# fatimp/SIFT3D

Measured on AMD Instinct MI355X. Metric: Mvoxel/s detect+describe (float32 volume resident in HBM), higher is better.
Workload: dtype f32; 1 GPU; 512x512x512 float32 lattice-blob volume, detect+describe, default parameters (sigma0 1.6, sigma_n 1.15, 3 levels/octave); parallelism=single GPU

## Files before the change

include/sift3d_amd.h:

```cpp
#ifndef SIFT3D_AMD_H
#define SIFT3D_AMD_H

#include <stddef.h>
#include <stdint.h>

#include "sift3d/imtypes.h"

#ifdef __cplusplus
extern "C" {
#endif

#define SIFT3D_AMD_API __attribute__((visibility("default")))


SIFT3D_AMD_API int
sift3d_amd_detect_keypoints_device(sift3d_detector *det, const float *d_volume,
                                   int nx, int ny, int nz, double ux, double uy,
                                   double uz, sift3d_keypoint_store *store);

SIFT3D_AMD_API int
sift3d_amd_image_set_units(sift3d_image *im, double ux, double uy, double uz);

SIFT3D_AMD_API int
sift3d_amd_detector_set_cuboid_extrema(sift3d_detector *det, int on);
// ... 308 lines not shown
SIFT3D_AMD_API int sift3d_hip_memcpy_d2d(void *d_dst, const void *d_src, size_t bytes, void *stream);
SIFT3D_AMD_API int sift3d_hip_memcpy2d_d2h(void *h_dst, size_t dst_pitch, const void *d_src,
                                           size_t src_pitch, size_t width, size_t height, void *stream);
SIFT3D_AMD_API int sift3d_hip_stream_wait_event(void *stream, void *ev);
SIFT3D_AMD_API int sift3d_hip_rows_scatter(float *d_dst, const void *d_all, size_t blk_bytes,
                                           const uint32_t *d_map, uint32_t n, void *stream);
SIFT3D_AMD_API int sift3d_hip_max_rows(float *d_dst, const float *d_rows, int nrows, int n, void *stream);
SIFT3D_AMD_API int sift3d_hip_memset(void *d_dst, int byte, size_t bytes, void *stream);
SIFT3D_AMD_API void *sift3d_hip_stream_create(void);
SIFT3D_AMD_API void *sift3d_hip_stream_create_high(void);
SIFT3D_AMD_API void sift3d_hip_stream_destroy(void *stream);
SIFT3D_AMD_API int sift3d_hip_stream_sync(void *stream);
SIFT3D_AMD_API void *sift3d_hip_event_create(void);
SIFT3D_AMD_API void sift3d_hip_event_destroy(void *ev);
SIFT3D_AMD_API int sift3d_hip_event_record(void *ev, void *stream);
SIFT3D_AMD_API double sift3d_hip_event_elapsed_ms(void *ev_start, void *ev_stop);


SIFT3D_AMD_API int
sift3d_hip_absmax(const float *d_src, size_t n, float *d_max, void *stream);

SIFT3D_AMD_API int
sift3d_hip_scale(const float *d_src, float *d_dst, size_t n, const float *d_max,
                 void *stream);

#define SIFT3D_HIP_MAX_TAPS 65

typedef struct {
    const float *src;
    float *dst;
    int nx, ny, nz;
    int axis;
    int width;
    const float *taps;
    float unit_factor;
    int n_glob, off;
    int z_lo, z_hi;
    int variant;
} sift3d_hip_fir_args;

SIFT3D_AMD_API int
sift3d_hip_fir(const sift3d_hip_fir_args *args, void *stream);
SIFT3D_AMD_API int
sift3d_hip_fir_x_scaled(const sift3d_hip_fir_args *args, const float *d_max, void *stream);
SIFT3D_AMD_API int sift3d_hip_fir_x_scaled_covers(const sift3d_hip_fir_args *args);

SIFT3D_AMD_API int
sift3d_hip_fir_yz_u1(const float *d_src, float *d_dst, int nx, int ny, int nz, const float *taps,
                     int width, int n_glob, int off, int z_lo, int z_hi, void *stream);
SIFT3D_AMD_API int sift3d_hip_fir_yz_u1_covers(const float *d_src, const float *d_dst, int nx, int ny,
                                               int width, int n_glob);

SIFT3D_AMD_API int
sift3d_hip_subtract_absmax(const float *d_a, const float *d_b, float *d_dst, size_t n,
                           float *d_absmax, void *stream);

#define SIFT3D_HIP_MAX_DOG_STACK 8
SIFT3D_AMD_API int sift3d_hip_dog_stack(const float *const *d_g, float *const *d_d, int n_gauss,
                                        size_t n, float *d_absmax, void *stream);

SIFT3D_AMD_API int
sift3d_hip_downsample2(const float *d_src, int nx, int ny, float *d_dst, int mx, int my,
                       int mz, void *stream);

typedef struct {
    const float *prev, *cur, *next;
    const float *d_absmax;
    int z_lo, z_hi;
    int tag;
} sift3d_hip_extrema_level;

typedef struct {
    uint32_t idx;
    int32_t tag;
    float val;
} sift3d_hip_cand;

SIFT3D_AMD_API size_t
sift3d_hip_extrema_work_bytes(int nx, int ny, int nz, int nlevels);
SIFT3D_AMD_API int
sift3d_hip_extrema(const sift3d_hip_extrema_level *levels, int nlevels, int nx, int ny,
                   int nz, double peak_thresh, sift3d_hip_cand *d_out, uint32_t cap,
                   uint32_t *d_count, void *d_work, size_t work_bytes, void *stream);

SIFT3D_AMD_API int
sift3d_hip_extrema_mode(const sift3d_hip_extrema_level *levels, int nlevels, int nx, int ny, int nz,
                        double peak_thresh, int cuboid, sift3d_hip_cand *d_out, uint32_t cap,
                        uint32_t *d_count, void *d_work, size_t work_bytes, void *stream);

SIFT3D_AMD_API int sift3d_hip_dogmax_stack(const float *const *d_g, int n_gauss, size_t n,
                                           float *d_absmax, void *stream);
SIFT3D_AMD_API int
sift3d_hip_extrema_gauss6(const float *const *d_g, const float *d_absmax, int nx, int ny, int nz,
                          int z_lo, int z_hi, int tag0, double peak_thresh, sift3d_hip_cand *d_out,
                          uint32_t cap, uint32_t *d_count, void *d_work, size_t work_bytes,
                          void *stream);
SIFT3D_AMD_API int
sift3d_hip_extrema_gauss6_phase(const float *const *d_g, const float *d_absmax, int nx, int ny, int nz,
                                int z_lo, int z_hi, int tag0, double peak_thresh, sift3d_hip_cand *d_out,
                                uint32_t cap, uint32_t *d_count, void *d_work, size_t work_bytes,
                                void *stream, int phase);
SIFT3D_AMD_API int sift3d_hip_dogmax_sub(const float *const *d_g, int nx, int ny, int nz, float *d_est,
                                         void *stream);
typedef struct {
    const float *const *d_g;
    int nx, ny, nz;
// ... 100 lines not shown
```

profiles/pmc_fir.py:

```python
#!/usr/bin/env python3
import csv
import glob
import json
import os
import sys

ROOT = os.path.dirname(os.path.dirname(os.path.abspath(__file__)))
sys.path.insert(0, ROOT)


def _require_built():
    lib = os.environ.get("SIFT3D_AMD_LIB") or os.path.join(ROOT, "sift3d_amd", "libsift3d_amd.so")
    if not os.path.exists(lib):
        sys.exit("%s is missing -- build first: python3 -c \"from sift3d_amd import _native; "
                 "_native.build()\"" % lib)

SIG = [0.5387011637869722, 0.9732939207323564, 1.2262734984654078, 1.5450077936447955,
       1.9465878414647133, 2.4525469969308156]


def run_guarded(*a, **k):
    _require_built()
    return run(*a, **k)


def run(n=512, reps=3):
    import torch
    from sift3d_amd import api, hip
    src = torch.empty((n, n, n), device="cuda")
    dst = torch.empty_like(src)
    hip.synth_lattice(src, 0, 11)
    for s in SIG:
        taps = api.gauss_filter(s)
        for ax in range(3):
            for _ in range(reps):
                hip.fir(src, dst, ax, taps)
        for _ in range(reps):
            hip.fir_yz(src, dst, taps)
    torch.cuda.synchronize()


def run_pyramid(n=512, builds=2):
    import torch
    from sift3d_amd import api, hip
    _require_built()
    vol = torch.empty((n, n, n), device="cuda")
    hip.synth_lattice(vol, 0, 11)
    torch.cuda.synchronize()
    det = api.Detector()
    for _ in range(builds):
        assert det.build_pyramid_device(vol.data_ptr(), n, n, n) == 0
    torch.cuda.synchronize()


def parse_pyramid(fetch_dir, write_dir, n=512, builds=2):
    def total(d, name):
        tot, by = 0.0, {}
        for f in glob.glob(os.path.join(d, "**", "*counter_collection.csv"), recursive=True):
            for r in csv.DictReader(open(f)):
                if r["Counter_Name"] != name or "synth" in r["Kernel_Name"]:
                    continue
                k = r["Kernel_Name"].split("(")[0].replace("void ", "")
                v = float(r["Counter_Value"])
                tot += v
                by[k] = by.get(k, 0.0) + v
        return tot, by
    fe, fby = total(fetch_dir, "FETCH_SIZE")
    wr, wby = total(write_dir, "WRITE_SIZE")
    num_oct = 0
    m = n
    alg = 0
    while m >= 8:
        alg += 24 * m ** 3 * (6 if num_oct == 0 else 5)
        num_oct += 1
        m //= 2
    hbm = (2.0 * fe + wr) * 1024.0 / builds
    by = {k: round((2.0 * fby.get(k, 0.0) + wby.get(k, 0.0)) * 1024.0 / builds) for k in set(fby) | set(wby)}
    return dict(hbm_bytes=round(hbm), algorithmic_bytes=alg, ratio=round(hbm / alg, 3), builds=builds,
                note="every kernel of sift3d_amd_build_pyramid_device (max|v|, all FIR passes of all octaves, "
                     "down-sampling): (2 * FETCH_SIZE + WRITE_SIZE) * 1024 summed over its dispatches",
                hbm_bytes_by_kernel=dict(sorted(by.items(), key=lambda kv: -kv[1])))


def parse(fetch_dir, write_dir, n=512):
    def load(d, name):
        out = {}
        for f in glob.glob(os.path.join(d, "**", "*counter_collection.csv"), recursive=True):
            for r in csv.DictReader(open(f)):
                if r["Counter_Name"] != name:
                    continue
                k = r["Kernel_Name"].split("(")[0].replace("void ", "")
                gx = int(r["Grid_Size_X"]) if "Grid_Size_X" in r else 0
                out.setdefault((k, gx), []).append(float(r["Counter_Value"]))
        return out
    fe, wr = load(fetch_dir, "FETCH_SIZE"), load(write_dir, "WRITE_SIZE")
    res = {}
    for (k, gx), v in fe.items():
        if "fir" not in k:
            continue
        w = wr.get((k, gx), [0.0])
        fetch_b = 2.0 * 1024.0 * sum(v) / len(v)
        write_b = 1024.0 * sum(w) / len(w)
        alg = (16 if "yz" in k else 8) * n ** 3
        res[k] = dict(fetch_bytes=round(fetch_b), write_bytes=round(write_b),
                      hbm_bytes=round(fetch_b + write_b), algorithmic_bytes=alg,
                      ratio=round((fetch_b + write_b) / float(alg), 3), dispatches=len(v))
    return res


if __name__ == "__main__":
    if len(sys.argv) > 1 and sys.argv[1] == "--parse":
        res = parse(sys.argv[2], sys.argv[3])
        if len(sys.argv) > 5:
            res["pyramid_build_512"] = parse_pyramid(sys.argv[4], sys.argv[5])
        print(json.dumps(res, indent=1, sort_keys=True))
    elif len(sys.argv) > 1 and sys.argv[1] == "--pyramid":
        run_pyramid()
    else:
        run_guarded()
```

sift3d_amd/csrc/sift3d_detect.c:

```c

static int require_device(void)
{
    if (!sift3d_amd_device_available()) {
        ERR("sift3d_amd: no HIP device is available; this library has no CPU path \n");
        return SIFT3D_FAILURE;
    }
    return SIFT3D_SUCCESS;
}

static int ensure_device(sift3d_detector *d)
{
    int i;
    if (d->stream) {
        if (sift3d_hip_current_device() != d->device) {
            ERR("sift3d_amd: this detector belongs to HIP device %d, the current device is %d \n",
                d->device, sift3d_hip_current_device());
            return SIFT3D_FAILURE;
        }
        return SIFT3D_SUCCESS;
    }
    if (require_device())
        return SIFT3D_FAILURE;
    d->device = sift3d_hip_current_device();
    if (!(d->stream = sift3d_hip_stream_create()) || !(d->oct_stream = sift3d_hip_stream_create_high()) ||
// ... 19 lines not shown
    return require_device() ? SIFT3D_FAILURE : upload_mesh();
}

static int ensure_cand_capacity(sift3d_detector *d, uint32_t cap)
{
    if (cap <= d->cand_cap)
        return SIFT3D_SUCCESS;
    free_cand_arrays(d);
    d->d_cand = (sift3d_hip_cand *)sift3d_hip_malloc(sizeof(sift3d_hip_cand) * (size_t)cap);
    d->h_cand = (sift3d_hip_cand *)sift3d_hip_host_alloc(sizeof(sift3d_hip_cand) * (size_t)cap);
    d->h_R = (float *)sift3d_hip_host_alloc(sizeof(float) * 9 * (size_t)cap);
    d->h_keep = (int32_t *)sift3d_hip_host_alloc(sizeof(int32_t) * ((size_t)cap + 4));
    if (!d->d_cand || !d->h_cand || !d->h_R || !d->h_keep)
        return SIFT3D_FAILURE;
    d->cand_cap = cap;
    return SIFT3D_SUCCESS;
}

static int stream_after(void *waiter, void *ev, void *src)
{
    return sift3d_hip_event_record(ev, src) || sift3d_hip_stream_wait_event(waiter, ev);
}

static inline float *dogmax_slot(const sift3d_detector *d, int o) { return d->d_scalars + 8 + o * d->ndl; }
static inline float *dogmax_bound_slot(const sift3d_detector *d, int o) { return dogmax_slot(d, d->num_octaves + o); }
static inline uint32_t *cand_counter(const sift3d_detector *d) { return (uint32_t *)(d->d_scalars + 1); }
static inline const float *const *octave_levels(const sift3d_detector *d, int o)
{
    return (const float *const *)(d->d_g + o * d->ngl);
}
static inline void *extrema_work(const sift3d_detector *d, int o, size_t *bytes)
{
    *bytes = o ? sift3d_hip_extrema_work_bytes(d->odims[o][0], d->odims[o][1], d->odims[o][2], 3) : d->work_bytes;
    return o ? (void *)((char *)d->d_work2 + d->work2_off[o]) : d->d_work;
}
static inline int dog_free_covers(const sift3d_detector *d, int o)
{
    return !d->cuboid_extrema && d->ngl == 6 && (d->odims[o][0] & 3) == 0 && d->odims[o][2] >= 3;
}
static inline int est_octave(const sift3d_detector *d, int o)
{
    return d->est0 && octave_voxels(d, o) >= ((size_t)1 << 21);
}

static int ensure_dog_octave(sift3d_detector *d, int o)
{
    const size_t n = octave_voxels(d, o);
    int s;
    for (s = 0; s < d->ndl; s++)
        if (!d->d_d[o * d->ndl + s] &&
            !(d->d_d[o * d->ndl + s] = (float *)sift3d_hip_malloc(n * sizeof(float))))
            return SIFT3D_FAILURE;
    return SIFT3D_SUCCESS;
}

static int fir_pass(const float *src, float *dst, const int *dims, const double *lu, const filter_t *f, int axis,
                    const float *d_scale_max, void *stream)
{
    sift3d_hip_fir_args a;
    memset(&a, 0, sizeof(a));
    a.src = src; a.dst = dst;
    a.nx = dims[0]; a.ny = dims[1]; a.nz = dims[2];
    a.axis = axis; a.width = f->width; a.taps = f->taps;
    a.unit_factor = (float)(1.0 / lu[axis]);
    a.n_glob = dims[2]; a.z_lo = 0; a.z_hi = dims[2];
    return d_scale_max ? sift3d_hip_fir_x_scaled(&a, d_scale_max, stream) : sift3d_hip_fir(&a, stream);
}

static int blur_level(sift3d_detector *d, const float *src, float *dst, const int *dims,
                      const double *lu, const filter_t *f, void *stream, float *tmp_a, float *tmp_b,
                      int slot, const float *d_scale_max)
{
    const float *in = src;
    float *outs[3] = { tmp_a, tmp_b, dst };
    int ax = 0;
    if ((float)(1.0 / lu[1]) == 1.0f && (float)(1.0 / lu[2]) == 1.0f) {
        int rc;
        if (!d || slot >= SIFT3D_AMD_TIMED_BLURS)
            slot = -1;
        if (slot >= 0)
            sift3d_hip_event_record(d->ev_blur[slot][0], stream);
        rc = fir_pass(src, tmp_a, dims, lu, f, 0, d_scale_max, stream);
        if (rc == 1 && d_scale_max)
            return 2;
        if (rc != SIFT3D_SUCCESS)
            return SIFT3D_FAILURE;
        if (slot >= 0)
            sift3d_hip_event_record(d->ev_blur[slot][1], stream);
        rc = sift3d_hip_fir_yz_u1_covers(tmp_a, dst, dims[0], dims[1], f->width, dims[2])
                 ? sift3d_hip_fir_yz_u1(tmp_a, dst, dims[0], dims[1], dims[2], f->taps, f->width, dims[2], 0, 0,
                                        dims[2], stream)
                 : 1;
        if (rc == SIFT3D_SUCCESS) {
            if (slot >= 0) {
                sift3d_hip_event_record(d->ev_blur[slot][2], stream);
                d->yz_timed |= 1u << slot;
            }
            return SIFT3D_SUCCESS;
        }
        if (rc != 1)
            return SIFT3D_FAILURE;
        in = tmp_a;
        ax = 1;
    } else if (d_scale_max) {
        return 2;
    }
    for (; ax < 3; ax++) {
        if (fir_pass(in, outs[ax], dims, lu, f, ax, NULL, stream))
            return SIFT3D_FAILURE;
        in = outs[ax];
    }
    return SIFT3D_SUCCESS;
}

#define HOST_THREADS_MAX 8
static int host_threads(size_t n)
{
    int t = omp_get_num_procs();
    if (t > HOST_THREADS_MAX)
        t = HOST_THREADS_MAX;
    if (n < 4096 || t < 1)
        t = 1;
    return t;
}

static int orient_scratch(sift3d_detector *d)
{
    const size_t need = sift3d_hip_orient_tab_bytes(d->num_octaves * d->ngl, d->cand_cap);
    if (need > d->otab_bytes) {
        sift3d_hip_free(d->d_otab);
        d->otab_bytes = 0;
        d->d_otab = sift3d_hip_malloc(need);
        if (!d->d_otab || sift3d_hip_memset(d->d_otab, 0, need, d->stream) || sift3d_hip_stream_sync(d->stream))
            return SIFT3D_FAILURE;
// ... 9 lines not shown
    if (!r_view || !k_view)
        return SIFT3D_FAILURE;
    return sift3d_hip_orient_tab_part(d->d_levels, d->num_octaves * d->ngl, lv_lo, lv_hi, d->d_cand, first, n,
                                      d->corner_thresh, r_view, k_view, d->orient_serial ? NULL : d->d_otab,
                                      d->cand_cap, slot, stream);
}

typedef struct {
    const float *vol;
    size_t n0;
    double t_start;
    int side;
    int ds;
    int forked, overlap;
    int im_stored;
    uint32_t count, count_a;
    int oriented;
} detect_run;

static int detect_begin(sift3d_detector *d, detect_run *r, const float *d_vol, int nx, int ny, int nz,
                        double ux, double uy, double uz)
{
    const int dims_changed = !d->have_im || d->nx != nx || d->ny != ny || d->nz != nz ||
                             !d->num_octaves;
    uint64_t rng;
    int o;
    memset(r, 0, sizeof(*r));
    r->t_start = now_s();
    r->vol = d_vol;
    r->n0 = (size_t)nx * ny * nz;

    d->have_im = 1;
    d->nx = nx; d->ny = ny; d->nz = nz;
    d->units[0] = ux; d->units[1] = uy; d->units[2] = uz;
    d->have_pyramid = 0;
    d->im_valid = 0;
    d->last_vol = NULL;
    d->t_pending &= ~1;
    if (dims_changed && resize_detector(d)) {
        d->have_im = 0;
        return SIFT3D_FAILURE;
    }
    fill_level_table(d);
    if (sift3d_hip_memcpy_h2d(d->d_levels, d->h_levels,
                              sizeof(sift3d_hip_level) * (size_t)d->num_octaves * d->ngl, d->stream))
        return SIFT3D_FAILURE;

    rng = range_start("sift3d: max|v|");
    sift3d_hip_event_record(d->ev[0], d->stream);
    if (sift3d_hip_memset(d->d_scalars, 0, sizeof(float) * (8 + 2 * (size_t)d->num_octaves * d->ndl), d->stream) ||
        sift3d_hip_absmax(d_vol, r->n0, d->d_scalars, d->stream))
        return SIFT3D_FAILURE;
    d->yz_timed = 0;
    d->parts_timed = 0;
    d->pyr_chains = 0;
    r->side = d->num_octaves > 1 && d->num_octaves <= 32 && d->d_work2;
    for (o = 0; o < d->num_octaves && r->side; o++)
        r->side = dog_free_covers(d, o);
    range_stop(rng);
    return SIFT3D_SUCCESS;
}

static int blur_levels(sift3d_detector *d, int o, int s_lo, int s_hi, void *stream, float *ta, float *tb)
{
    double lu[3];
    int s;
    level_units(d, o, lu);
    for (s = s_lo; s < s_hi; s++)
        if (blur_level(d, d->d_g[o * d->ngl + s - 1], d->d_g[o * d->ngl + s], d->odims[o], lu, &d->filt[s],
                       stream, ta, tb, o == 0 ? s : -1, NULL))
            return SIFT3D_FAILURE;
    return SIFT3D_SUCCESS;
}

static int downsample_octave(sift3d_detector *d, const detect_run *r, int o, void *stream)
{
    return sift3d_hip_downsample2(d->d_g[o * d->ngl + r->ds + 1], d->odims[o][0], d->odims[o][1],
                                  d->d_g[(o + 1) * d->ngl], d->odims[o + 1][0], d->odims[o + 1][1],
                                  d->odims[o + 1][2], stream);
}

static int first_blur(sift3d_detector *d, detect_run *r)
{
    double lu[3];
    int rc;
    level_units(d, 0, lu);
    rc = blur_level(d, r->vol, d->d_g[0], d->odims[0], lu, &d->filt[0], d->stream, d->d_tmp_a, d->d_tmp_b, 0,
                    d->d_scalars);
    if (rc == 2) {
        if (sift3d_hip_scale(r->vol, d->d_im, r->n0, d->d_scalars, d->stream) ||
            blur_level(d, d->d_im, d->d_g[0], d->odims[0], lu, &d->filt[0], d->stream, d->d_tmp_a, d->d_tmp_b,
                       0, NULL))
            return SIFT3D_FAILURE;
        r->im_stored = 1;
        return SIFT3D_SUCCESS;
    }
    return rc;
}

static int build_forked_octaves(sift3d_detector *d, const detect_run *r)
{
    const int rest = r->ds + 2;
    int o;
    if (blur_levels(d, 0, 1, rest, d->stream, d->d_tmp_a, d->d_tmp_b) ||
        stream_after(d->oct_stream, d->ev_fork, d->stream) || downsample_octave(d, r, 0, d->oct_stream))
        return SIFT3D_FAILURE;
// ... 660 lines not shown
```

sift3d_amd/csrc/sift3d_host.c:

```c
#include <float.h>
#include <math.h>
#include <stdint.h>
#include <stdio.h>
#include <stdlib.h>
#include <string.h>
#include <time.h>
#include <zlib.h>
#include <omp.h>
#include <dlfcn.h>
#include <pthread.h>

#include "../../include/sift3d/imutil.h"
#include "../../include/sift3d/sift.h"
#include "../../include/sift3d_amd.h"

#define ERR(...) fprintf(stderr, __VA_ARGS__)

#define NFACES 20
#define NVERT 12
#define DESC_NUMEL 768
#define SLAB_LEN 500

static const double peak_thresh_default = 0.1;
static const int num_kp_levels_default = 3;
// ... 16 lines not shown
    int num_cols, num_rows;
    sift3d_mat_type type;
};

typedef struct {
    float R[9];
    double xd, yd, zd, sd;
    int o, s;
    float strength;
} keypoint_t;

struct _sift3d_keypoint_store {
    keypoint_t *buf;
    size_t num, cap;
    int nx, ny, nz;
};

struct _sift3d_descriptor_store {
    float *hist;
    double *xyzsd;
    size_t num, cap;
    int pinned;
    int keep_device;
    float *d_hist;
    size_t d_cap, d_num;
    int nx, ny, nz;
};

typedef struct {
    double sigma;
    int width;
    float *taps;
} filter_t;

struct _sift3d_detector {
    double peak_thresh, corner_thresh, sigma_n, sigma0;
    int cuboid_extrema;
    int num_kp_levels;
    int have_im;
    int nx, ny, nz;
    double units[3];
    double alloc_units[3];
    int num_octaves, ngl, ndl;
    int (*odims)[3];
    filter_t *filt;
    int nfilt;
    void *stream;
    void *oct_stream;
    void *side_stream;
    void *ev_fork, *ev_join, *ev_join2, *ev_part;
    int parts_timed;
    void *ev_blur[SIFT3D_AMD_TIMED_BLURS][3];
    unsigned yz_timed;
    void *ev_pyr[2];
    int pyr_chains;
    void *ev_oct[32];
    int device;
    void *ev[8];
    float *d_im, *d_tmp_a, *d_tmp_b, *d_in;
    float *d_tmp2_a, *d_tmp2_b;
    float *d_tmp3_a, *d_tmp3_b;
    size_t in_cap;
    float **d_g, **d_d;
    unsigned char dog_free[64];
    float *d_scalars;
    int t_pending;
    int orient_serial;
    int exact_desc;
    int im_valid;
    const float *last_vol;
    int est0;
    sift3d_hip_level *h_levels, *d_levels;
    sift3d_hip_cand *d_cand, *h_cand;
    uint32_t cand_cap;
    uint32_t cand_cap0;
    float *h_R;
    int32_t *h_keep;
    void *d_work;
    size_t work_bytes;
    void *d_work2;
    size_t work2_off[64], work2_bytes;
    float *d_wlut;
    void *d_dpart;
    size_t dpart_bytes;
    void *d_otab;
    size_t otab_bytes;
    sift3d_hip_kp *h_kp;
    uint32_t kp_cap;
    int have_pyramid;
    int ncand;
    double t[SIFT3D_AMD_NUM_TIMINGS];
};

enum {
    T_UPLOAD, T_PYRAMID, T_DOG, T_EXTREMA, T_ORIENT, T_DESCRIBE, T_PYRAMID_DEV, T_DETECT_WALL, T_DESCRIBE_WALL, T_LAST_YZ,
    T_BLUR_X,
    T_BLUR_YZ = T_BLUR_X + SIFT3D_AMD_TIMED_BLURS,
    T_DETECT_DEV = T_BLUR_YZ + SIFT3D_AMD_TIMED_BLURS, T_COMPACT, T_ORIENT_OCT0_END, T_ORIENT_REST_END, T_COUNT
};
typedef char timing_slots_match_the_header[T_COUNT == SIFT3D_AMD_NUM_TIMINGS ? 1 : -1];

static pthread_mutex_t g_mesh_lock = PTHREAD_MUTEX_INITIALIZER;
static unsigned char g_mesh_ready[64];

static double now_s(void)
{
// ... 1037 lines not shown
    int i;
    if (!d)
        return;
    if (d->stream)
        sift3d_hip_stream_sync(d->stream);
    free_device_pyramid(d);
    free_filters(d);
    sift3d_hip_free(d->d_in);
    free_cand_arrays(d);
    sift3d_hip_host_free(d->h_kp);
    for (i = 0; i < 8; i++)
        sift3d_hip_event_destroy(d->ev[i]);
    sift3d_hip_event_destroy(d->ev_fork);
    sift3d_hip_event_destroy(d->ev_join);
    sift3d_hip_event_destroy(d->ev_join2);
    sift3d_hip_event_destroy(d->ev_part);
    for (i = 0; i < SIFT3D_AMD_TIMED_BLURS * 3; i++)
        sift3d_hip_event_destroy(d->ev_blur[i / 3][i % 3]);
    sift3d_hip_event_destroy(d->ev_pyr[0]);
    sift3d_hip_event_destroy(d->ev_pyr[1]);
    for (i = 0; i < 32; i++)
        sift3d_hip_event_destroy(d->ev_oct[i]);
    sift3d_hip_stream_destroy(d->side_stream);
    sift3d_hip_stream_destroy(d->oct_stream);
    sift3d_hip_stream_destroy(d->stream);
    free(d);
}

static double stage_seconds(void *a, void *b)
{
    const double ms = sift3d_hip_event_elapsed_ms(a, b);
    return ms >= 0.0 ? 1e-3 * ms : (double)NAN;
}

const double *sift3d_amd_timings(const sift3d_detector *dc)
{
    sift3d_detector *d = (sift3d_detector *)dc;
    if (d->t_pending & 1) {
        d->t[T_UPLOAD] = stage_seconds(d->ev[0], d->ev[1]);
        int b, last = -1;
        d->t[T_PYRAMID] = stage_seconds(d->ev[1], d->ev[2]);
        if (d->pyr_chains)
            for (b = 0; b < 2; b++) {
                const double tc = stage_seconds(d->ev[1], d->ev_pyr[b]);
                if (tc > d->t[T_PYRAMID] || isnan(tc))
                    d->t[T_PYRAMID] = tc;
            }
        d->t[T_DOG] = stage_seconds(d->ev[2], d->ev[3]);
        d->t[T_EXTREMA] = stage_seconds(d->ev[3], d->ev[4]);
        d->t[T_ORIENT] = stage_seconds(d->ev[4], d->ev[5]);
        d->t[T_PYRAMID_DEV] = d->t[T_PYRAMID];
        for (b = 0; b < SIFT3D_AMD_TIMED_BLURS; b++) {
            const int on = (d->yz_timed >> b) & 1;
            d->t[T_BLUR_X + b] = on ? stage_seconds(d->ev_blur[b][0], d->ev_blur[b][1]) : 0.0;
            d->t[T_BLUR_YZ + b] = on ? stage_seconds(d->ev_blur[b][1], d->ev_blur[b][2]) : 0.0;
            if (on)
                last = b;
        }
        d->t[T_LAST_YZ] = last >= 0 ? d->t[T_BLUR_YZ + last] : 0.0;
        d->t[T_DETECT_DEV] = stage_seconds(d->ev[0], d->ev[5]);
        d->t[T_ORIENT_OCT0_END] = d->parts_timed ? stage_seconds(d->ev[0], d->ev_part) : 0.0;
        d->t[T_ORIENT_REST_END] = d->parts_timed ? stage_seconds(d->ev[0], d->ev_join) : 0.0;
    }
    if (d->t_pending & 2)
        d->t[T_DESCRIBE] = stage_seconds(d->ev[6], d->ev[7]);
    d->t_pending = 0;
    return d->t;
}
int sift3d_amd_num_candidates(const sift3d_detector *d) { return d->ncand; }

int sift3d_amd_describe_clock(const sift3d_detector *d, double *cycles, double *seconds)
{
    uint64_t c = 0, t = 0;
    if (!d || !d->d_wlut || !d->num_octaves || !cycles || !seconds ||
        sift3d_hip_describe_clock(d->d_wlut, d->num_octaves * d->ngl, 0, &c, &t, d->stream))
        return SIFT3D_FAILURE;
    *cycles = (double)c;
    *seconds = (double)t * 1e-8;
    return SIFT3D_SUCCESS;
}

int sift3d_amd_detector_dogmax(const sift3d_detector *d, float *out, int cap)
{
    const int n = d ? d->num_octaves * d->ndl : 0;
    if (!d || !out || !d->have_pyramid || !d->d_scalars || n < 1 || cap < n)
        return -1;
    if (sift3d_hip_memcpy_d2h(out, d->d_scalars + 8, sizeof(float) * (size_t)n, d->stream) ||
        sift3d_hip_stream_sync(d->stream))
        return -1;
    return n;
}

static struct {
    pthread_once_t once;
    uint64_t (*start)(const char *);
    void (*stop)(uint64_t);
} g_roctx = { PTHREAD_ONCE_INIT, NULL, NULL };

static void roctx_load(void)
{
    static const char *names[] = { "librocprofiler-sdk-roctx.so.1", "librocprofiler-sdk-roctx.so",
                                   "libroctx64.so.4", "libroctx64.so" };
    void *lib = NULL;
    size_t i;
    const char *e = getenv("SIFT3D_AMD_ROCTX");
    if (e && e[0] == '0')
        return;
    for (i = 0; i < sizeof(names) / sizeof(names[0]) && !lib; i++)
// ... 86 lines not shown
```

sift3d_amd/hip.py:

```python
import ctypes as C

import numpy as np

from . import _native

MAX_TAPS = 65
FACE_FLOATS = 19


class FirArgs(C.Structure):
    _fields_ = [("src", C.c_void_p), ("dst", C.c_void_p), ("nx", C.c_int), ("ny", C.c_int),
                ("nz", C.c_int), ("axis", C.c_int), ("width", C.c_int),
                ("taps", C.POINTER(C.c_float)), ("unit_factor", C.c_float), ("n_glob", C.c_int),
                ("off", C.c_int), ("z_lo", C.c_int), ("z_hi", C.c_int), ("variant", C.c_int)]


class ExtremaLevel(C.Structure):
    _fields_ = [("prev", C.c_void_p), ("cur", C.c_void_p), ("next", C.c_void_p),
                ("d_absmax", C.c_void_p), ("z_lo", C.c_int), ("z_hi", C.c_int), ("tag", C.c_int)]


class Level(C.Structure):
    _fields_ = [("data", C.c_void_p), ("nx", C.c_int), ("ny", C.c_int), ("nz", C.c_int),
                ("z_off", C.c_int), ("nz_glob", C.c_int), ("ux", C.c_float), ("uy", C.c_float),
                ("uz", C.c_float), ("octave", C.c_int), ("sd", C.c_double)]


class DemonsLevel(C.Structure):
    _fields_ = [("d_F", C.c_void_p), ("nx", C.c_int), ("ny", C.c_int), ("nz", C.c_int), ("d_M", C.c_void_p),
                ("mx", C.c_int), ("my", C.c_int), ("mz", C.c_int), ("iterations", C.c_int)]


CAND_DTYPE = np.dtype([("idx", "u4"), ("tag", "i4"), ("val", "f4")])
KP_DTYPE = np.dtype([("R", "f4", (9,)), ("cx", "f4"), ("cy", "f4"), ("cz", "f4"),
                     ("level", "i4"), ("row1", "u4"), ("sd", "f8")], align=True)
LEVEL_DTYPE = np.dtype([("data", "u8"), ("nx", "i4"), ("ny", "i4"), ("nz", "i4"),
                        ("z_off", "i4"), ("nz_glob", "i4"), ("ux", "f4"), ("uy", "f4"),
                        ("uz", "f4"), ("octave", "i4"), ("sd", "f8")], align=True)
assert LEVEL_DTYPE.itemsize == C.sizeof(Level)
assert KP_DTYPE.itemsize == 64 and CAND_DTYPE.itemsize == 12

_bound = None


def lib():
    global _bound
    if _bound is not None:
        return _bound
    L = _native.load()
    vp = C.c_void_p
    sig = {
        "sift3d_hip_device_count": (C.c_int, []),
        "sift3d_hip_set_device": (C.c_int, [C.c_int]),
        "sift3d_hip_malloc": (vp, [C.c_size_t]),
        "sift3d_hip_free": (None, [vp]),
        "sift3d_hip_host_alloc": (vp, [C.c_size_t]),
        "sift3d_hip_host_free": (None, [vp]),
        "sift3d_hip_memcpy_h2d": (C.c_int, [vp, vp, C.c_size_t, vp]),
        "sift3d_hip_memcpy_d2h": (C.c_int, [vp, vp, C.c_size_t, vp]),
        "sift3d_hip_memcpy_d2d": (C.c_int, [vp, vp, C.c_size_t, vp]),
        "sift3d_hip_memset": (C.c_int, [vp, C.c_int, C.c_size_t, vp]),
        "sift3d_hip_stream_create": (vp, []),
        "sift3d_hip_stream_destroy": (None, [vp]),
        "sift3d_hip_stream_sync": (C.c_int, [vp]),
        "sift3d_hip_event_create": (vp, []),
        "sift3d_hip_event_destroy": (None, [vp]),
        "sift3d_hip_event_record": (C.c_int, [vp, vp]),
        "sift3d_hip_event_elapsed_ms": (C.c_double, [vp, vp]),
        "sift3d_hip_absmax": (C.c_int, [vp, C.c_size_t, vp, vp]),
        "sift3d_hip_scale": (C.c_int, [vp, vp, C.c_size_t, vp, vp]),
        "sift3d_hip_fir": (C.c_int, [C.POINTER(FirArgs), vp]),
        "sift3d_hip_fir_yz_u1": (C.c_int, [vp, vp, C.c_int, C.c_int, C.c_int, C.POINTER(C.c_float),
                                          C.c_int, C.c_int, C.c_int, C.c_int, C.c_int, vp]),
        "sift3d_hip_nn2_work_floats": (C.c_size_t, [C.c_int, C.c_int]),
        "sift3d_hip_nn2": (C.c_int, [vp, C.c_int, vp, C.c_int, C.c_int, vp, vp, vp, vp, vp]),
        "sift3d_hip_subtract_absmax": (C.c_int, [vp, vp, vp, C.c_size_t, vp, vp]),
        "sift3d_hip_dog_stack": (C.c_int, [C.POINTER(vp), C.POINTER(vp), C.c_int, C.c_size_t, vp, vp]),
        "sift3d_hip_dogmax_stack": (C.c_int, [C.POINTER(vp), C.c_int, C.c_size_t, vp, vp]),
        "sift3d_hip_host_device_ptr": (vp, [vp]),
        "sift3d_hip_downsample2": (C.c_int, [vp, C.c_int, C.c_int, vp, C.c_int, C.c_int, C.c_int, vp]),
        "sift3d_hip_extrema_work_bytes": (C.c_size_t, [C.c_int, C.c_int, C.c_int, C.c_int]),
        "sift3d_hip_extrema": (C.c_int, [C.POINTER(ExtremaLevel), C.c_int, C.c_int, C.c_int, C.c_int,
                                         C.c_double, vp, C.c_uint32, vp, vp, C.c_size_t, vp]),
        "sift3d_hip_extrema_mode": (C.c_int, [C.POINTER(ExtremaLevel), C.c_int, C.c_int, C.c_int, C.c_int,
                                              C.c_double, C.c_int, vp, C.c_uint32, vp, vp, C.c_size_t, vp]),
        "sift3d_hip_orient": (C.c_int, [vp, vp, C.c_uint32, C.c_double, vp, vp, vp]),
        "sift3d_hip_orient_tab_bytes": (C.c_size_t, [C.c_int, C.c_uint32]),
        "sift3d_hip_orient_tab": (C.c_int, [vp, C.c_int, vp, C.c_uint32, C.c_double, vp, vp, vp, C.c_uint32, vp]),
        "sift3d_hip_orient_tab_part": (C.c_int, [vp, C.c_int, C.c_int, C.c_int, vp, C.c_uint32, C.c_uint32,
                                                 C.c_double, vp, vp, vp, C.c_uint32, C.c_int, vp]),
        "sift3d_hip_describe": (C.c_int, [vp, vp, C.c_uint32, vp, vp]),
        "sift3d_hip_set_mesh": (C.c_int, [C.POINTER(C.c_float)]),
        "sift3d_hip_synth_lattice": (C.c_int, [vp, C.c_int, C.c_int, C.c_int, C.c_int, C.c_uint64, vp]),
        "sift3d_hip_warp_affine": (C.c_int, [vp, C.c_int, C.c_int, C.c_int, vp, C.c_int, C.c_int, C.c_int,
                                             C.POINTER(C.c_double), C.c_int, C.c_float, vp]),
        "sift3d_hip_warp_tps": (C.c_int, [vp, C.c_int, C.c_int, C.c_int, vp, C.c_int, C.c_int, C.c_int,
                                          C.POINTER(C.c_double), vp, C.c_int, C.c_int, C.c_float, vp]),
        "sift3d_hip_warp_tps_launches": (C.c_int, [C.c_int, C.c_int, C.c_int, C.c_int]),
        "sift3d_hip_affine_field": (C.c_int, [vp, C.c_int, C.c_int, C.c_int, C.POINTER(C.c_double), vp]),
        "sift3d_hip_tps_field": (C.c_int, [vp, C.c_int, C.c_int, C.c_int, C.POINTER(C.c_double), vp, C.c_int, vp]),
        "sift3d_hip_tps_field_launches": (C.c_int, [C.c_int, C.c_int, C.c_int, C.c_int]),
        "sift3d_hip_warp_field": (C.c_int, [vp, C.c_int, C.c_int, C.c_int, C.c_int, vp, C.c_int, C.c_int, C.c_int,
                                            vp, C.c_int, C.c_float, vp]),
        "sift3d_hip_jacobian_det": (C.c_int, [vp, C.c_int, C.c_int, C.c_int, vp, vp, vp]),
        "sift3d_hip_bspline_work_floats": (C.c_size_t, [C.c_int, C.c_int, C.c_int]),
        "sift3d_hip_bspline_prefilter": (C.c_int, [vp, C.c_int, C.c_int, C.c_int, C.c_int, vp, vp, vp]),
        "sift3d_hip_bspline_warp_affine": (C.c_int, [vp, C.c_int, C.c_int, C.c_int, vp, C.c_int, C.c_int, C.c_int,
                                                     C.POINTER(C.c_double), C.c_float, vp]),
        "sift3d_hip_bspline_warp_field": (C.c_int, [vp, C.c_int, C.c_int, C.c_int, C.c_int, vp, C.c_int, C.c_int,
                                                    C.c_int, vp, C.c_float, vp]),
        "sift3d_amd_similarity_work_bytes": (C.c_size_t, [C.c_int, C.c_int, C.c_int, C.c_int]),
        "sift3d_hip_similarity_affine": (C.c_int, [vp, C.c_int, C.c_int, C.c_int, vp, C.c_int, C.c_int, C.c_int,
                                                   C.POINTER(C.c_double), C.c_int, C.c_int, C.c_float, C.c_float,
                                                   C.c_float, C.c_float, vp, vp, vp, vp]),
        "sift3d_hip_similarity_field": (C.c_int, [vp, C.c_int, C.c_int, C.c_int, vp, C.c_int, C.c_int, C.c_int, vp,
                                                  C.c_int, C.c_int, C.c_float, C.c_float, C.c_float, C.c_float, vp, vp,
                                                  vp, vp]),
        "sift3d_hip_dense_bin": (C.c_int, [vp, C.c_int, C.c_int, C.c_int, C.c_double, C.c_double, C.c_double,
                                           vp, vp]),
        "sift3d_hip_dense_normalize": (C.c_int, [vp, C.c_size_t, vp]),
        "sift3d_amd_dense_work_floats": (C.c_size_t, [C.c_int, C.c_int, C.c_int]),
        "sift3d_amd_dense_descriptors_device": (C.c_int, [vp, C.c_int, C.c_int, C.c_int, C.POINTER(C.c_double),
                                                          C.c_double, vp, vp, vp]),
        "sift3d_hip_dense_orient": (C.c_int, [vp, C.c_int, C.c_int, C.c_int, C.c_double, C.c_double, C.c_double,
                                              C.c_double, vp, vp, vp]),
        "sift3d_hip_dense_rotate_bin": (C.c_int, [vp, C.c_int, C.c_int, C.c_int, C.c_double, C.c_double,
# ... 25 lines not shown
        "sift3d_hip_test_expf": (C.c_int, [vp, vp, C.c_size_t, vp]),
        "sift3d_hip_test_eigen3": (C.c_int, [vp, vp, vp, C.c_size_t, vp]),
        "sift3d_hip_last_error": (C.c_char_p, []),
    }
    for name, (res, args) in sig.items():
        fn = getattr(L, name)
        fn.restype = res
        fn.argtypes = args
    _bound = L
    return L


def _check(rc, what):
    if rc != 0:
        raise RuntimeError("%s failed: %s" % (what, lib().sift3d_hip_last_error().decode()))


_stream = None


def current_stream(refresh=False):
    global _stream
    if _stream is None or refresh:
        import torch
        _stream = C.c_void_p(torch.cuda.current_stream().cuda_stream)
    return _stream


def fir(src, dst, axis, taps, unit_factor=1.0, n_glob=None, off=0, z_lo=0, z_hi=None, variant=0):
    nz, ny, nx = src.shape
    assert src.is_contiguous() and dst.is_contiguous() and src.shape == dst.shape
    taps = np.ascontiguousarray(taps, np.float32)
    a = FirArgs(src.data_ptr(), dst.data_ptr(), nx, ny, nz, axis, len(taps),
                taps.ctypes.data_as(C.POINTER(C.c_float)), float(np.float32(unit_factor)),
                nz if n_glob is None else n_glob, off, z_lo, nz if z_hi is None else z_hi, variant)
    _check(lib().sift3d_hip_fir(C.byref(a), current_stream()), "sift3d_hip_fir")
    return dst


def fir_yz(src, dst, taps, n_glob=None, off=0, z_lo=0, z_hi=None):
    nz, ny, nx = src.shape
    assert src.is_contiguous() and dst.is_contiguous() and src.shape == dst.shape
    taps = np.ascontiguousarray(taps, np.float32)
    rc = lib().sift3d_hip_fir_yz_u1(src.data_ptr(), dst.data_ptr(), nx, ny, nz,
                                    taps.ctypes.data_as(C.POINTER(C.c_float)), len(taps),
                                    nz if n_glob is None else n_glob, off, z_lo,
                                    nz if z_hi is None else z_hi, current_stream())
    if rc == 1:
        return False
    _check(rc, "sift3d_hip_fir_yz_u1")
    return True


def nn2(a, b):
    import torch
    assert a.is_contiguous() and b.is_contiguous() and a.shape[1] == b.shape[1]
    na, nb = a.shape[0], b.shape[0]
    j = torch.empty(max(na, 1), dtype=torch.int32, device=a.device)
    d1 = torch.empty(max(na, 1), dtype=torch.float32, device=a.device)
    d2 = torch.empty_like(d1)
    work = torch.empty(lib().sift3d_hip_nn2_work_floats(na, nb), dtype=torch.float32, device=a.device)
    _check(lib().sift3d_hip_nn2(a.data_ptr(), na, b.data_ptr(), nb, a.shape[1], j.data_ptr(),
                                d1.data_ptr(), d2.data_ptr(), work.data_ptr(), current_stream()),
           "sift3d_hip_nn2")
    return j[:na], d1[:na], d2[:na]


INTERP = {"nearest": 0, "linear": 1}


def _interp(interp):
    if interp not in INTERP:
        raise ValueError("interp must be 'nearest' or 'linear', not %r" % (interp,))
    return INTERP[interp]


def _tensor(t, msg, dims=None, lead=None, shape=None, device=None, dtype="float32"):
    import torch
    if not (isinstance(t, torch.Tensor) and t.is_cuda and (dtype is None or t.dtype == getattr(torch, dtype))
            and t.is_contiguous() and (dims is None or t.dim() in dims)
            and (lead is None or (t.dim() >= 1 and t.shape[0] == lead))
            and (shape is None or tuple(t.shape) == tuple(shape)) and (device is None or t.device == device)):
        raise ValueError(msg)


def _field_tensor(t, what, name="field"):
    _tensor(t, "%s: %s must be a contiguous float32 CUDA tensor [3, oz, oy, ox]" % (what, name), dims=(4,), lead=3)


def _same_device(what, *ts):
    if any(t.device != ts[0].device for t in ts):
        raise ValueError("%s: the tensors are not on one device" % what)


def _work(work, need, like, what, dtype=None):
    import torch
    if work is None:
        return torch.empty(need, dtype=torch.float32, device=like.device)
    _tensor(work, "%s: work must be a contiguous %sCUDA tensor of >= %d bytes on the device of the other tensors"
            % (what, dtype + " " if dtype else "", 4 * need), device=like.device, dtype=dtype)
    if work.numel() * work.element_size() < 4 * need:
        raise ValueError("%s: work holds fewer than %d bytes" % (what, 4 * need))
    return work


def _warp_pair(src, dst, what):
# ... 647 lines not shown
```

Before: 4049 Mvoxel/s.

## Fuse x, y and z Gaussian FIR passes into one LDS-staged kernel

```diff
diff --git a/include/sift3d_amd.h b/include/sift3d_amd.h
--- a/include/sift3d_amd.h
+++ b/include/sift3d_amd.h
@@ -384,6 +384,12 @@
                                                int width, int n_glob);
 
 SIFT3D_AMD_API int
+sift3d_hip_fir_xyz(const float *d_src, float *d_dst, int nx, int ny, int nz, const float *taps, int width,
+                   const float *d_scale_max, void *stream);
+SIFT3D_AMD_API int sift3d_hip_fir_xyz_covers(const float *d_src, const float *d_dst, int nx, int ny, int nz,
+                                             int width, float uf_x, float uf_y, float uf_z);
+
+SIFT3D_AMD_API int
 sift3d_hip_subtract_absmax(const float *d_a, const float *d_b, float *d_dst, size_t n,
                            float *d_absmax, void *stream);
 
diff --git a/profiles/pmc_fir.py b/profiles/pmc_fir.py
--- a/profiles/pmc_fir.py
+++ b/profiles/pmc_fir.py
@@ -14,6 +14,8 @@
     if not os.path.exists(lib):
         sys.exit("%s is missing -- build first: python3 -c \"from sift3d_amd import _native; "
                  "_native.build()\"" % lib)
+
+FUSED_HW = (2, 3, 4, 5)
 
 SIG = [0.5387011637869722, 0.9732939207323564, 1.2262734984654078, 1.5450077936447955,
        1.9465878414647133, 2.4525469969308156]
@@ -37,6 +39,8 @@
                 hip.fir(src, dst, ax, taps)
         for _ in range(reps):
             hip.fir_yz(src, dst, taps)
+        for _ in range(reps):
+            hip.fir_xyz(src, dst, taps)
     torch.cuda.synchronize()
 
 
@@ -101,10 +105,15 @@
         w = wr.get((k, gx), [0.0])
         fetch_b = 2.0 * 1024.0 * sum(v) / len(v)
         write_b = 1024.0 * sum(w) / len(w)
-        alg = (16 if "yz" in k else 8) * n ** 3
+        alg = (24 if "xyz" in k else 16 if "yz" in k else 8) * n ** 3
         res[k] = dict(fetch_bytes=round(fetch_b), write_bytes=round(write_b),
                       hbm_bytes=round(fetch_b + write_b), algorithmic_bytes=alg,
                       ratio=round((fetch_b + write_b) / float(alg), 3), dispatches=len(v))
+    for hw in FUSED_HW:
+        ty = 64 if hw <= 2 else 32
+        slot, one = "k_fir_yz_dma<%d, %d>" % (hw, ty), "k_fir_xyz_dma<%d, %d, false>" % (hw, ty)
+        if one in res:
+            res[slot] = dict(res[one], launched=one, yz_pass_hbm_bytes=res.get(slot, {}).get("hbm_bytes"))
     return res
 
 
diff --git a/sift3d_amd/csrc/sift3d_detect.c b/sift3d_amd/csrc/sift3d_detect.c
--- a/sift3d_amd/csrc/sift3d_detect.c
+++ b/sift3d_amd/csrc/sift3d_detect.c
@@ -95,6 +95,13 @@
             !(d->d_d[o * d->ndl + s] = (float *)sift3d_hip_malloc(n * sizeof(float))))
             return SIFT3D_FAILURE;
     return SIFT3D_SUCCESS;
+}
+
+#define FIR_XYZ_WINS 0x3Cu
+#define FIR_XYZ_MIN_VOXELS ((size_t)256 * 256 * 256)
+static int fir_xyz_wins(int hw, size_t voxels)
+{
+    return hw >= 1 && hw <= 8 && ((FIR_XYZ_WINS >> hw) & 1) && voxels >= FIR_XYZ_MIN_VOXELS;
 }
 
 static int fir_pass(const float *src, float *dst, const int *dims, const double *lu, const filter_t *f, int axis,
@@ -123,6 +130,18 @@
             slot = -1;
         if (slot >= 0)
             sift3d_hip_event_record(d->ev_blur[slot][0], stream);
+        if (d && fir_xyz_wins(f->width / 2, (size_t)dims[0] * dims[1] * dims[2]) &&
+            sift3d_hip_fir_xyz_covers(src, dst, dims[0], dims[1], dims[2], f->width, (float)(1.0 / lu[0]),
+                                      (float)(1.0 / lu[1]), (float)(1.0 / lu[2]))) {
+            if (sift3d_hip_fir_xyz(src, dst, dims[0], dims[1], dims[2], f->taps, f->width, d_scale_max, stream))
+                return SIFT3D_FAILURE;
+            if (slot >= 0) {
+                sift3d_hip_event_record(d->ev_blur[slot][2], stream);
+                d->yz_timed |= 1u << slot;
+                d->xyz_timed |= 1u << slot;
+            }
+            return SIFT3D_SUCCESS;
+        }
         rc = fir_pass(src, tmp_a, dims, lu, f, 0, d_scale_max, stream);
         if (rc == 1 && d_scale_max)
             return 2;
@@ -238,6 +257,7 @@
         sift3d_hip_absmax(d_vol, r->n0, d->d_scalars, d->stream))
         return SIFT3D_FAILURE;
     d->yz_timed = 0;
+    d->xyz_timed = 0;
     d->parts_timed = 0;
     d->pyr_chains = 0;
     r->side = d->num_octaves > 1 && d->num_octaves <= 32 && d->d_work2;
diff --git a/sift3d_amd/csrc/sift3d_fir_xyz.hip b/sift3d_amd/csrc/sift3d_fir_xyz.hip
--- /dev/null
+++ b/sift3d_amd/csrc/sift3d_fir_xyz.hip
@@ -0,0 +1,340 @@
+#include "sift3d_kernels_common.h"
+
+#include <atomic>
+
+template <int HW, int TY> struct XyzGeom {
+    static constexpr int TXQ = 16, SQ = 20, HALO = 8, W = 2 * HW + 1, ROWS = TY + 2 * HW, NB = 4;
+    static constexpr int NT = 16 * TY, NWAVE = NT / 64;
+    static constexpr int NQ = ROWS * SQ;
+    static constexpr int NP = (NQ + 63) / 64;
+    static constexpr int TILEQ = NP * 64;
+    static constexpr int SEQ = 320;
+    static constexpr size_t LDS_BYTES = (size_t)(NB * TILEQ + ROWS * TXQ) * 16 + (SEQ + 1) * 4;
+    static_assert((NP + NWAVE - 1) / NWAVE == 2, "two pieces per wave and request");
+    static_assert(HW <= HALO, "halo too small");
+};
+
+template <int HW, int TY, bool SCALED>
+__global__ __launch_bounds__(16 * TY) __attribute__((amdgpu_waves_per_eu(4, 4))) void k_fir_xyz_dma(
+    FirParams P, FirTaps T, EdgeTab Ex, EdgeTab Ey, EdgeTab Ez)
+{
+    typedef XyzGeom<HW, TY> G;
+    constexpr int TXQ = G::TXQ, SQ = G::SQ, HALO = G::HALO, W = G::W, ROWS = G::ROWS, NB = G::NB, NT = G::NT;
+    constexpr int NWAVE = G::NWAVE, NQ = G::NQ, NP = G::NP, TILEQ = G::TILEQ, SEQ = G::SEQ;
+    extern __shared__ float4 smem[];
+    float4 *const stg = smem;
+    float4 *const xf = smem + NB * TILEQ;
+    int *const seq = reinterpret_cast<int *>(xf + ROWS * TXQ);
+    const int tid = threadIdx.x;
+    const int wave = __builtin_amdgcn_readfirstlane(tid >> 6), lane = tid & 63;
+    const int qx = tid % TXQ, ty = tid / TXQ;
+    const int x0 = blockIdx.x * (4 * TXQ);
+    const int x = x0 + qx * 4;
+    const int y0 = blockIdx.y * TY;
+    const int y = y0 + ty;
+    const int nx = P.nx, ny = P.ny;
+    const size_t plane = (size_t)nx * ny;
+    const int nl1 = P.nz - 1;
+    const int endz = nl1, endy = ny - 1, endx = nx - 1;
+    const int p0 = blockIdx.z * P.ts;
+    const int p1 = min(p0 + P.ts, P.nz);
+
+    if (tid == 0) {
+        int n = 0;
+        for (int i = p0 - HW; i < p1 + HW && n + 2 <= SEQ; i++) {
+            if (i < 0) {
+                seq[n++] = clampi(-i, 0, nl1);
+            } else if (i >= endz) {
+                const int m = i - endz;
+                if (m <= HW) {
+                    int lo = 0;
+                    for (int mm = 0; mm <= HW; mm++)
+                        lo = mm == m ? Ez.lo[mm] : lo;
+                    seq[n++] = clampi(lo, 0, nl1);
+                    seq[n++] = clampi(lo + 1, 0, nl1);
+                }
+            } else {
+                seq[n++] = i;
+            }
+        }
+        seq[SEQ] = n;
+    }
+    __syncthreads();
+    const int nreq = __builtin_amdgcn_readfirstlane(seq[SEQ]);
+
+    size_t srcoff[2];
+    uint32_t pcoff[2];
+#pragma unroll
+    for (int k = 0; k < 2; k++) {
+        const int pc = min(NWAVE * k + wave, NP - 1);
+        const int f = 64 * pc + lane;
+        const int j = min(f / SQ, ROWS - 1);
+        const int i = y0 - HW + j;
+        const int sr = i < 0 ? min(-i, endy) : min(i, endy);
+        const int xq = clampi(x0 - HALO + 4 * (f % SQ), 0, nx - 4);
+        srcoff[k] = (size_t)sr * nx + xq;
+        pcoff[k] = (uint32_t)__builtin_amdgcn_readfirstlane(pc * 1024);
+    }
+    const uint32_t lds0 = (uint32_t)(uintptr_t)(__attribute__((address_space(3))) float4 *)stg;
+    auto stage = [&](int t) {
+        const int pl = __builtin_amdgcn_readfirstlane(seq[min(t, nreq - 1)]);
+        const float *src = P.src + (size_t)pl * plane;
+        const uint32_t tb = lds0 + (uint32_t)((t & (NB - 1)) * (TILEQ * 16));
+        unsigned keep;
+#pragma unroll
+        for (int k = 0; k < 2; k++) {
+            const float *g = src + srcoff[k];
+            const uint32_t dst = (uint32_t)__builtin_amdgcn_readfirstlane((int)(tb + pcoff[k]));
+            asm volatile("s_mov_b32 %0, m0\n\ts_mov_b32 m0, %2\n\ts_nop 0\n\tglobal_load_lds_dwordx4 %1, off\n\ts_mov_b32 m0, %0"
+                         : "=&s"(keep) : "v"(g), "s"(dst) : "memory");
+        }
+    };
+    auto wait_barrier = [&](int n) {
+        switch (n) {
+        case 4: asm volatile("s_waitcnt vmcnt(4)\n\ts_barrier" ::: "memory"); break;
+        case 5: asm volatile("s_waitcnt vmcnt(5)\n\ts_barrier" ::: "memory"); break;
+        case 6: asm volatile("s_waitcnt vmcnt(6)\n\ts_barrier" ::: "memory"); break;
+        default: asm volatile("s_waitcnt vmcnt(7)\n\ts_barrier" ::: "memory"); break;
+        }
+    };
+    auto lds_barrier = [&]() { asm volatile("s_waitcnt lgkmcnt(0)\n\ts_barrier" ::: "memory"); };
+
+    const bool xlo = blockIdx.x == 0, xhi = blockIdx.x == gridDim.x - 1;
+    const int xe = tid & 15;
+    int xpos = 0;
+    float xw0 = 0.0f, xw1 = 0.0f;
+#pragma unroll
+    for (int mm = 0; mm <= HW; mm++)
+        if (mm == xe) {
+            xpos = clampi(Ex.lo[mm], 0, endx - 1) - x0 + HALO;
+            xw0 = Ex.w0[mm];
+            xw1 = Ex.w1[mm];
+        }
+    xpos = clampi(xpos, 0, 4 * SQ - 2);
+    const bool yedge = y0 + TY + HW > endy;
+    const int em = tid >> 4;
+    const int ej = endy + em - (y0 - HW);
+    const bool efix = yedge && em <= HW && ej < ROWS;
+    int elo = 0;
+    float ew0 = 0.0f, ew1 = 0.0f;
+#pragma unroll
+    for (int mm = 0; mm <= HW; mm++)
+        if (mm == em) {
+            elo = Ey.lo[mm] - (y0 - HW);
+            ew0 = Ey.w0[mm];
+            ew1 = Ey.w1[mm];
+        }
+    float smax = 1.0f;
+    if (SCALED) {
+        smax = *P.scale_max;
+        smax = smax != 0.0f ? smax : 1.0f;
+    }
+    int t = 0;
+    int shist = 0;
+    stage(0);
+    stage(1);
+    stage(2);
+    auto xyfilt = [&]() -> float4 {
+        wait_barrier(4 + __builtin_popcount(shist));
+        stage(t + NB - 1);
+        float4 *const tile = stg + (t & (NB - 1)) * TILEQ;
+        if (SCALED) {
+            for (int f = tid; f < NQ; f += NT) {
+                float4 q = tile[f];
+                q.x = q.x / smax; q.y = q.y / smax; q.z = q.z / smax; q.w = q.w / smax;
+                tile[f] = q;
+            }
+            lds_barrier();
+        }
+        if (xlo || xhi) {
+            for (int r = tid >> 4; r < ROWS; r += TY) {
+                float *const row = reinterpret_cast<float *>(tile + r * SQ);
+                if (xlo && xe < HALO)
+                    row[HALO - 1 - xe] = row[HALO + 1 + xe];
+                if (xhi && xe <= HW) {
+                    const float a = row[xpos], c = row[xpos + 1];
+                    row[HALO + 4 * TXQ - 1 + xe] = xw0 * a + xw1 * c;
+                }
+            }
+            lds_barrier();
+        }
+#pragma unroll
+        for (int k = 0; k < 2; k++) {
+            const int r = ty + k * TY;
+            if (r < ROWS) {
+                float w[4 + 2 * HALO];
+#pragma unroll
+                for (int i = 0; i < (4 + 2 * HALO) / 4; i++) {
+                    const float4 q = tile[r * SQ + qx + i];
+                    w[4 * i] = q.x; w[4 * i + 1] = q.y; w[4 * i + 2] = q.z; w[4 * i + 3] = q.w;
+                }
+                float o[4];
+#pragma unroll
+                for (int c = 0; c < 4; c++) {
+                    float acc = 0.0f;
+#pragma unroll
+                    for (int dd = -HW; dd <= HW; dd++)
+                        acc += T.k[dd + HW] * w[HALO + c - dd];
+                    o[c] = acc;
+                }
+                xf[r * TXQ + qx] = make_float4(o[0], o[1], o[2], o[3]);
+            }
+        }
+        lds_barrier();
+        if (yedge) {
+            if (efix) {
+                const float4 a = xf[clampi(elo, 0, ROWS - 1) * TXQ + qx], c = xf[clampi(elo + 1, 0, ROWS - 1) * TXQ + qx];
+                xf[ej * TXQ + qx] = Vec<4>::lerp(ew0, a, ew1, c);
+            }
+            lds_barrier();
+        }
+        float4 acc = make_float4(0.f, 0.f, 0.f, 0.f);
+#pragma unroll
+        for (int dd = -HW; dd <= HW; dd++)
+            Vec<4>::mac(acc, T.k[dd + HW], xf[(ty + HW - dd) * TXQ + qx]);
+        t++;
+        return acc;
+    };
+    auto ext_z = [&](int i, bool stores) -> float4 {
+        if (HW < 6 && i < endz) {
+            const float4 yv = xyfilt();
+            shist = ((shist << 1) | (int)stores) & 7;
+            return yv;
+        }
+        int np = 1;
+        float w0 = 1.0f, w1 = 0.0f;
+        if (i >= endz) {
+            const int m = i - endz;
+            np = m > HW ? 0 : 2;
+#pragma unroll
+            for (int mm = 0; mm <= HW; mm++)
+                if (mm == m) {
+                    w0 = Ez.w0[mm];
+                    w1 = Ez.w1[mm];
+                }
+        }
+        float4 a = make_float4(0.f, 0.f, 0.f, 0.f);
+#pragma unroll 1
+        for (int k = 0; k < np; k++) {
+            const float4 yv = xyfilt();
+            shist = ((shist << 1) | (int)(stores && k + 1 == np)) & 7;
+            if (k == 0)
+                a = yv;
+            else
+                a = Vec<4>::lerp(w0, a, w1, yv);
+        }
+        if (np == 0)
+            shist = ((shist << 1) | (int)stores) & 7;
+        return a;
+    };
+
+    float4 ring[W];
+#pragma unroll
+    for (int i = 0; i < W; i++)
+        ring[i] = make_float4(0.f, 0.f, 0.f, 0.f);
+#pragma unroll
+    for (int i = 0; i < 2 * HW; i++)
+        ring[i] = ext_z(p0 - HW + i, false);
+    float *__restrict__ d = P.dst + (size_t)y * nx + x;
+#pragma unroll 1
+    for (int q0 = p0; q0 < p1; q0 += W) {
+#pragma unroll
+        for (int j = 0; j < W; j++) {
+            const int q = q0 + j;
+            if (q < p1) {
+                ring[(j + 2 * HW) % W] = ext_z(q + HW, true);
+                float4 acc = make_float4(0.f, 0.f, 0.f, 0.f);
+#pragma unroll
+                for (int dd = -HW; dd <= HW; dd++)
+                    Vec<4>::mac(acc, T.k[dd + HW], ring[(j + HW - dd) % W]);
+                st4(d + (size_t)q * plane, acc);
+            }
+        }
+    }
+    asm volatile("s_waitcnt vmcnt(0)" ::: "memory");
+}
+
+template <int HW, int TY, bool SCALED>
+static hipError_t launch_fir_xyz_t(const FirParams &P, const FirTaps &T, const EdgeTab &Ex, const EdgeTab &Ey,
+                                   const EdgeTab &Ez, int nseg, hipStream_t st)
+{
+    typedef XyzGeom<HW, TY> G;
+    auto kern = k_fir_xyz_dma<HW, TY, SCALED>;
+    static std::atomic<unsigned long long> allowed{0};
+    int dev = 0;
+    hipError_t e = hipGetDevice(&dev);
+    if (e != hipSuccess)
+        return e;
+    if (dev < 0 || dev >= 64 || !((allowed.load(std::memory_order_relaxed) >> dev) & 1)) {
+        e = hipFuncSetAttribute(reinterpret_cast<const void *>(kern), hipFuncAttributeMaxDynamicSharedMemorySize,
+                                (int)G::LDS_BYTES);
+        if (e != hipSuccess)
+            return e;
+        if (dev >= 0 && dev < 64)
+            allowed.fetch_or(1ull << dev, std::memory_order_relaxed);
+    }
+    hipLaunchKernelGGL(kern, dim3(P.nx / 64, P.ny / TY, nseg), dim3(G::NT), G::LDS_BYTES, st, P, T, Ex, Ey, Ez);
+    return hipSuccess;
+}
+
+template <int HW>
+static hipError_t launch_fir_xyz(const FirParams &P, const FirTaps &T, const EdgeTab &Ex, const EdgeTab &Ey,
+                                 const EdgeTab &Ez, int nseg, hipStream_t st)
+{
+    constexpr int DTY = HW <= 2 ? 64 : 32;
+    return P.scale_max ? launch_fir_xyz_t<HW, DTY, true>(P, T, Ex, Ey, Ez, nseg, st)
+                       : launch_fir_xyz_t<HW, DTY, false>(P, T, Ex, Ey, Ez, nseg, st);
+}
+
+extern "C" {
+
+int sift3d_hip_fir_xyz_covers(const float *d_src, const float *d_dst, int nx, int ny, int nz, int width,
+                              float uf_x, float uf_y, float uf_z)
+{
+    const int hw = width / 2;
+    return d_src && d_dst && d_src != d_dst && (width & 1) && hw >= 1 && hw <= 8 && uf_x == 1.0f && uf_y == 1.0f &&
+           uf_z == 1.0f && nx >= 64 && (nx & 63) == 0 && (ny & 63) == 0 && ny >= 128 && nz >= 1 && nz < (1 << 22) &&
+           ny < (1 << 22) && nx < (1 << 22) && ((((uintptr_t)d_src | (uintptr_t)d_dst) & 15) == 0);
+}
+
+int sift3d_hip_fir_xyz(const float *d_src, float *d_dst, int nx, int ny, int nz, const float *taps, int width,
+                       const float *d_scale_max, void *stream)
+{
+    hipStream_t st = (hipStream_t)stream;
+    const int hw = width / 2;
+    if (!d_src || !d_dst || !taps || nx < 1 || ny < 1 || nz < 1 || width < 1)
+        return launch_fail("sift3d_hip_fir_xyz", "invalid arguments");
+    if (!sift3d_hip_fir_xyz_covers(d_src, d_dst, nx, ny, nz, width, 1.0f, 1.0f, 1.0f))
+        return 1;
+    if (overlap(d_src, sizeof(float) * (size_t)nx * ny * nz, d_dst, sizeof(float) * (size_t)nx * ny * nz))
+        return launch_fail("sift3d_hip_fir_xyz", "source and destination overlap");
+    FirParams P;
+    FirTaps T;
+    memset(&T, 0, sizeof(T));
+    memcpy(T.k, taps, sizeof(float) * width);
+    memset(&P, 0, sizeof(P));
+    P.src = d_src; P.dst = d_dst;
+    P.nx = nx; P.ny = ny; P.nz = nz;
+    P.axis = 2; P.hw = hw; P.uf = 1.0f; P.uhw = hw;
+    P.n_glob = nz; P.z_hi = nz;
+    P.scale_max = d_scale_max;
+    long nseg;
+    {
+        const long blocks_xy = (long)(nx / 64) * (ny / 32);
+        const long want = (512 + blocks_xy - 1) / blocks_xy;
+        const long cap = nz / 32 > 1 ? nz / 32 : 1;
+        nseg = want < cap ? want : cap;
+        if ((nz + nseg - 1) / nseg > 256)
+            nseg = (nz + 255) / 256;
+        P.ts = (int)((nz + nseg - 1) / nseg);
+        nseg = (nz + P.ts - 1) / P.ts;
+    }
+    const EdgeTab Ex = edge_table(nx, hw), Ey = edge_table(ny, hw), Ez = edge_table(nz, hw);
+    hipError_t e = hipSuccess;
+    dispatch_int_or<1, 8, 8>(hw, [&](auto H) { e = launch_fir_xyz<decltype(H)::value>(P, T, Ex, Ey, Ez, (int)nseg, st); });
+    HIPCHK(e);
+    LAUNCH_CHECK();
+    return SIFT3D_SUCCESS;
+}
+
+}
diff --git a/sift3d_amd/csrc/sift3d_host.c b/sift3d_amd/csrc/sift3d_host.c
--- a/sift3d_amd/csrc/sift3d_host.c
+++ b/sift3d_amd/csrc/sift3d_host.c
@@ -92,6 +92,7 @@
     int parts_timed;
     void *ev_blur[SIFT3D_AMD_TIMED_BLURS][3];
     unsigned yz_timed;
+    unsigned xyz_timed;
     void *ev_pyr[2];
     int pyr_chains;
     void *ev_oct[32];
@@ -1235,8 +1236,9 @@
         d->t[T_PYRAMID_DEV] = d->t[T_PYRAMID];
         for (b = 0; b < SIFT3D_AMD_TIMED_BLURS; b++) {
             const int on = (d->yz_timed >> b) & 1;
-            d->t[T_BLUR_X + b] = on ? stage_seconds(d->ev_blur[b][0], d->ev_blur[b][1]) : 0.0;
-            d->t[T_BLUR_YZ + b] = on ? stage_seconds(d->ev_blur[b][1], d->ev_blur[b][2]) : 0.0;
+            const int one = (d->xyz_timed >> b) & 1;
+            d->t[T_BLUR_X + b] = on && !one ? stage_seconds(d->ev_blur[b][0], d->ev_blur[b][1]) : 0.0;
+            d->t[T_BLUR_YZ + b] = on ? stage_seconds(d->ev_blur[b][one ? 0 : 1], d->ev_blur[b][2]) : 0.0;
             if (on)
                 last = b;
         }
diff --git a/sift3d_amd/hip.py b/sift3d_amd/hip.py
--- a/sift3d_amd/hip.py
+++ b/sift3d_amd/hip.py
@@ -72,6 +72,10 @@
         "sift3d_hip_fir": (C.c_int, [C.POINTER(FirArgs), vp]),
         "sift3d_hip_fir_yz_u1": (C.c_int, [vp, vp, C.c_int, C.c_int, C.c_int, C.POINTER(C.c_float),
                                           C.c_int, C.c_int, C.c_int, C.c_int, C.c_int, vp]),
+        "sift3d_hip_fir_xyz": (C.c_int, [vp, vp, C.c_int, C.c_int, C.c_int, C.POINTER(C.c_float), C.c_int, vp, vp]),
+        "sift3d_hip_fir_xyz_covers": (C.c_int, [vp, vp, C.c_int, C.c_int, C.c_int, C.c_int, C.c_float, C.c_float,
+                                               C.c_float]),
+        "sift3d_hip_fir_x_scaled": (C.c_int, [C.POINTER(FirArgs), vp, vp]),
         "sift3d_hip_nn2_work_floats": (C.c_size_t, [C.c_int, C.c_int]),
         "sift3d_hip_nn2": (C.c_int, [vp, C.c_int, vp, C.c_int, C.c_int, vp, vp, vp, vp, vp]),
         "sift3d_hip_subtract_absmax": (C.c_int, [vp, vp, vp, C.c_size_t, vp, vp]),
@@ -203,6 +207,35 @@
     return True
 
 
+def fir_xyz(src, dst, taps, scale_max=None, unit_factors=(1.0, 1.0, 1.0)):
+    nz, ny, nx = src.shape
+    assert src.is_contiguous() and dst.is_contiguous() and src.shape == dst.shape
+    taps = np.ascontiguousarray(taps, np.float32)
+    if tuple(unit_factors) != (1.0, 1.0, 1.0) and not lib().sift3d_hip_fir_xyz_covers(
+            src.data_ptr(), dst.data_ptr(), nx, ny, nz, len(taps), *[float(np.float32(u)) for u in unit_factors]):
+        return False
+    rc = lib().sift3d_hip_fir_xyz(src.data_ptr(), dst.data_ptr(), nx, ny, nz,
+                                  taps.ctypes.data_as(C.POINTER(C.c_float)), len(taps),
+                                  None if scale_max is None else scale_max.data_ptr(), current_stream())
+    if rc == 1:
+        return False
+    _check(rc, "sift3d_hip_fir_xyz")
+    return True
+
+
+def fir_x_scaled(src, dst, taps, scale_max):
+    nz, ny, nx = src.shape
+    assert src.is_contiguous() and dst.is_contiguous() and src.shape == dst.shape
+    taps = np.ascontiguousarray(taps, np.float32)
+    a = FirArgs(src.data_ptr(), dst.data_ptr(), nx, ny, nz, 0, len(taps),
+                taps.ctypes.data_as(C.POINTER(C.c_float)), 1.0, nz, 0, 0, nz, 0)
+    rc = lib().sift3d_hip_fir_x_scaled(C.byref(a), scale_max.data_ptr(), current_stream())
+    if rc == 1:
+        return False
+    _check(rc, "sift3d_hip_fir_x_scaled")
+    return True
+
+
 def nn2(a, b):
     import torch
     assert a.is_contiguous() and b.is_contiguous() and a.shape[1] == b.shape[1]
```

After: 4110 Mvoxel/s (median of 6 runs). +1.5%, better.
